# chengruiz/cusrl

Hardware: AMD Instinct MI355X
Metric: env_steps_per_sec (higher is better)
Workload: dtype f32; 1 GPU; synthetic continuous env 4096x obs48 x act12 per GPU, MLP(256,128) actor-critic, rollout_len=24, ppo preset (5 epochs x 4 minibatches, Adam lr 2e-4); envs_per_gpu=4096, parallelism=dp1, rccl_ranks=0, collectives=none (single process), hipgraph=True, fused_env=True, captured_env_steps=24, epoch_graph_updates=432, unjoined_steps_captured=20, autoreset=False

## Files before the change

### cusrl_amd/csrc/mlp_forward.hip

```cpp
#include "common.hpp"

namespace cusrl {

typedef float mfma_f32x4 __attribute__((ext_vector_type(4)));

constexpr int kMlpWaves = 4;
constexpr int kMlpThreads = kMlpWaves * kWave;
constexpr int kMlpRows = 16;

struct MlpForwardArgs {
    const float *x;
    const float *w1, *b1, *w2, *b2, *w3, *b3;
    float *out;
    const float *std;
    const float *eps;
    float *action, *logp, *std_out;
    int64_t rows;
    int K, A;
};

__device__ __forceinline__ float log_sqrt_2pi_f() { return 0.91893853320467274178f; }

__device__ __forceinline__ mfma_f32x4 relu4(mfma_f32x4 v) {
    v[0] = v[0] <= 0.f ? 0.f : v[0], v[1] = v[1] <= 0.f ? 0.f : v[1], v[2] = v[2] <= 0.f ? 0.f : v[2], v[3] = v[3] <= 0.f ? 0.f : v[3];
    return v;
}

template <int T1, int T2, int KB>
__global__ __launch_bounds__(kMlpThreads) void mlp2_forward_kernel(const MlpForwardArgs p) {
    constexpr int NT1 = kMlpWaves * T1;
    __shared__ float4 hidden[NT1][kWave];
    __shared__ float4 partial[kMlpWaves][kWave];
    const int lane = threadIdx.x & (kWave - 1), wave = threadIdx.x / kWave;
    const int i = lane & 15, kk = lane >> 4;
    const int K = p.K, A = p.A;
    constexpr int H1 = 16 * NT1, H2 = 16 * kMlpWaves * T2;
    const float4 zero4 = make_float4(0.f, 0.f, 0.f, 0.f);

    float4 a1[T1][KB], a2[T2][NT1], a3[T2];
    mfma_f32x4 c1[T1], c2[T2], c3;
#pragma unroll
    for (int t1 = 0; t1 < T1; ++t1) {
        const int n = 16 * (T1 * wave + t1);
#pragma unroll
        for (int t = 0; t < KB; ++t) {
            const int k = 16 * t + 4 * kk;
            const float4 v = *reinterpret_cast<const float4 *>(p.w1 + int64_t(n + i) * K + (k < K ? k : 0));
            a1[t1][t] = k < K ? v : zero4;
        }
        const float4 b = *reinterpret_cast<const float4 *>(p.b1 + n + 4 * kk);
        c1[t1] = mfma_f32x4{b.x, b.y, b.z, b.w};
    }
    const int64_t tiles = (p.rows + kMlpRows - 1) / kMlpRows;
    float4 ahead[KB];
    auto request = [&](int64_t tile) {
        const int64_t row = min(tile * kMlpRows + i, p.rows - 1);
#pragma unroll
        for (int t = 0; t < KB; ++t) {
            const int k = 16 * t + 4 * kk;
            ahead[t] = *reinterpret_cast<const float4 *>(p.x + row * K + (k < K ? k : 0));
        }
    };
    request(min(int64_t(blockIdx.x), tiles - 1));
#pragma unroll
    for (int t2 = 0; t2 < T2; ++t2) {
        const int n = 16 * (T2 * wave + t2);
#pragma unroll
        for (int t = 0; t < NT1; ++t) a2[t2][t] = *reinterpret_cast<const float4 *>(p.w2 + int64_t(n + i) * H1 + 16 * t + 4 * kk);
        const float4 b = *reinterpret_cast<const float4 *>(p.b2 + n + 4 * kk);
        c2[t2] = mfma_f32x4{b.x, b.y, b.z, b.w};
        const float4 v = *reinterpret_cast<const float4 *>(p.w3 + int64_t(i < A ? i : 0) * H2 + n + 4 * kk);
        a3[t2] = i < A ? v : zero4;
    }
    c3 = mfma_f32x4{0.f, 0.f, 0.f, 0.f};
    if (wave == 0 && p.b3) {
#pragma unroll
        for (int reg = 0; reg < 4; ++reg) c3[reg] = 4 * kk + reg < A ? p.b3[4 * kk + reg] : 0.f;
    }

    float sigma[4] = {1.f, 1.f, 1.f, 1.f}, noise[4] = {0.f, 0.f, 0.f, 0.f};
    const bool sampling = wave == 0 && p.eps != nullptr;
    if (sampling) {
#pragma unroll
        for (int reg = 0; reg < 4; ++reg) sigma[reg] = p.std[min(4 * kk + reg, A - 1)];
    }

    for (int64_t tile = blockIdx.x; tile < tiles; tile += gridDim.x) {
        const int64_t row0 = tile * kMlpRows;
        if (sampling) {
            const int64_t first = min(row0 + i, p.rows - 1) * A;
#pragma unroll
            for (int reg = 0; reg < 4; ++reg) noise[reg] = p.eps[first + min(4 * kk + reg, A - 1)];
        }
        float4 xb[KB];
#pragma unroll
        for (int t = 0; t < KB; ++t) xb[t] = 16 * t + 4 * kk < K ? ahead[t] : zero4;
        request(min(tile + gridDim.x, tiles - 1));
#pragma unroll
        for (int t1 = 0; t1 < T1; ++t1) {
            mfma_f32x4 acc = c1[t1];
#pragma unroll
            for (int t = 0; t < KB; ++t) {
                const float av[4] = {a1[t1][t].x, a1[t1][t].y, a1[t1][t].z, a1[t1][t].w};
                const float bv[4] = {xb[t].x, xb[t].y, xb[t].z, xb[t].w};
#pragma unroll
                for (int j = 0; j < 4; ++j) acc = __builtin_amdgcn_mfma_f32_16x16x4f32(av[j], bv[j], acc, 0, 0, 0);
            }
            acc = relu4(acc);
            hidden[T1 * wave + t1][lane] = make_float4(acc[0], acc[1], acc[2], acc[3]);
        }
        __syncthreads();
        mfma_f32x4 h2[T2];
#pragma unroll
        for (int t2 = 0; t2 < T2; ++t2) h2[t2] = c2[t2];
#pragma unroll
        for (int t = 0; t < NT1; ++t) {
            const float4 hb = hidden[t][lane];
            const float bv[4] = {hb.x, hb.y, hb.z, hb.w};
#pragma unroll
            for (int j = 0; j < 4; ++j)
#pragma unroll
                for (int t2 = 0; t2 < T2; ++t2) {
                    const float av = j == 0 ? a2[t2][t].x : j == 1 ? a2[t2][t].y : j == 2 ? a2[t2][t].z : a2[t2][t].w;
                    h2[t2] = __builtin_amdgcn_mfma_f32_16x16x4f32(av, bv[j], h2[t2], 0, 0, 0);
                }
        }
        mfma_f32x4 head = c3;
#pragma unroll
        for (int t2 = 0; t2 < T2; ++t2) {
            const mfma_f32x4 h = relu4(h2[t2]);
            const float av[4] = {a3[t2].x, a3[t2].y, a3[t2].z, a3[t2].w};
#pragma unroll
            for (int j = 0; j < 4; ++j) head = __builtin_amdgcn_mfma_f32_16x16x4f32(av[j], h[j], head, 0, 0, 0);
        }
        partial[wave][lane] = make_float4(head[0], head[1], head[2], head[3]);
        __syncthreads();
        if (wave == 0) {
            float4 sum = partial[0][lane];
#pragma unroll
            for (int w = 1; w < kMlpWaves; ++w) {
                const float4 v = partial[w][lane];
                sum.x += v.x, sum.y += v.y, sum.z += v.z, sum.w += v.w;
            }
            const bool live = row0 + i < p.rows;
            const int a0 = 4 * kk;
            const int64_t at = (row0 + i) * A + a0;
            const float mu[4] = {sum.x, sum.y, sum.z, sum.w};
            if (live && p.out) {
                if (A % 4 == 0) {
                    if (a0 < A) *reinterpret_cast<float4 *>(p.out + at) = sum;
                } else {
#pragma unroll
                    for (int reg = 0; reg < 4; ++reg)
                        if (a0 + reg < A) p.out[at + reg] = mu[reg];
                }
            }
            if (p.eps) {
                float term[4] = {0.f, 0.f, 0.f, 0.f};
#pragma unroll
                for (int reg = 0; reg < 4; ++reg) {
                    const int a = a0 + reg;
                    if (a < A) {
                        const float sg = sigma[reg];
                        const float act = mu[reg] + noise[reg] * sg;
                        const float diff = act - mu[reg];
                        term[reg] = -(diff * diff) / (2.0f * (sg * sg)) - logf(sg) - log_sqrt_2pi_f();
                        if (live) {
                            p.action[at + reg] = act;
                            if (p.std_out) p.std_out[at + reg] = sg;
                        }
                    }
                }
                float lp = 0.f;
#pragma unroll
                for (int src = 0; src < 4; ++src)
#pragma unroll
                    for (int reg = 0; reg < 4; ++reg) {
                        const float t = __shfl(term[reg], i + 16 * src, kWave);
                        if (4 * src + reg < A) lp += t;
                    }
                if (live && kk == 0) p.logp[row0 + i] = lp;
            }
        }
    }
}

template <int T1, int T2>
static int launch_mlp2(const MlpForwardArgs &p, int kb, dim3 grid, hipStream_t s) {
    switch (kb) {
        case 1: hipLaunchKernelGGL((mlp2_forward_kernel<T1, T2, 1>), grid, dim3(kMlpThreads), 0, s, p); break;
        case 2: hipLaunchKernelGGL((mlp2_forward_kernel<T1, T2, 2>), grid, dim3(kMlpThreads), 0, s, p); break;
        case 3: hipLaunchKernelGGL((mlp2_forward_kernel<T1, T2, 3>), grid, dim3(kMlpThreads), 0, s, p); break;
        case 4: hipLaunchKernelGGL((mlp2_forward_kernel<T1, T2, 4>), grid, dim3(kMlpThreads), 0, s, p); break;
        default: return CUSRL_E_UNSUPPORTED;
    }
    return launch_status();
}

}

using namespace cusrl;

extern "C" int cusrl_mlp2_forward_supported(int64_t in_features, int64_t hidden1, int64_t hidden2, int64_t out_features) {
    return in_features >= 4 && in_features % 4 == 0 && in_features <= 64 && (hidden1 == 128 || hidden1 == 256) &&
           (hidden2 == 64 || hidden2 == 128) && out_features >= 1 && out_features <= 16;
}

extern "C" int cusrl_mlp2_forward(const float *input, int64_t rows, int64_t in_features, const float *w1, const float *b1,
                                  int64_t hidden1, const float *w2, const float *b2, int64_t hidden2, const float *w3,
                                  const float *b3, int64_t out_features, float *output, const float *std, const float *eps,
                                  float *action, float *logp, float *std_out, void *stream) {
    if (rows < 0 || !input || !w1 || !b1 || !w2 || !b2 || !w3) return CUSRL_E_INVALID;
    if (rows == 0) return 0;
    if (!cusrl_mlp2_forward_supported(in_features, hidden1, hidden2, out_features)) return CUSRL_E_UNSUPPORTED;
    const bool sampling = eps != nullptr;
    if (sampling ? !(std && action && logp) : (std || action || logp || std_out)) return CUSRL_E_INVALID;
    if (!sampling && !output) return CUSRL_E_INVALID;
    if (!aligned(input, 16) || !aligned(w1, 16) || !aligned(b1, 16) || !aligned(w2, 16) || !aligned(b2, 16) || !aligned(w3, 16) ||
        (output && out_features % 4 == 0 && !aligned(output, 16)))
        return CUSRL_E_UNSUPPORTED;
    MlpForwardArgs p;
    p.x = input, p.w1 = w1, p.b1 = b1, p.w2 = w2, p.b2 = b2, p.w3 = w3, p.b3 = b3, p.out = output;
    p.std = std, p.eps = eps, p.action = action, p.logp = logp, p.std_out = std_out;
    p.rows = rows, p.K = int(in_features), p.A = int(out_features);
    const int64_t tiles = ceil_div(rows, kMlpRows);
    static int cus = 0;
    if (cus == 0) {
        int device = 0, count = 0;
        if (hipGetDevice(&device) != hipSuccess || hipDeviceGetAttribute(&count, hipDeviceAttributeMultiprocessorCount, device) != hipSuccess || count <= 0)
            count = 256;
        cus = count;
    }
    const dim3 grid(uint32_t(tiles < cus ? tiles : cus));
    const int kb = int(ceil_div(in_features, 16));
    hipStream_t s = as_stream(stream);
    if (hidden1 == 256 && hidden2 == 128) return launch_mlp2<4, 2>(p, kb, grid, s);
    if (hidden1 == 256 && hidden2 == 64) return launch_mlp2<4, 1>(p, kb, grid, s);
    if (hidden1 == 128 && hidden2 == 128) return launch_mlp2<2, 2>(p, kb, grid, s);
    return launch_mlp2<2, 1>(p, kb, grid, s);
}
```

### cusrl_amd/hook/on_policy/value.py

```python

from __future__ import annotations

import torch
from torch import Tensor, nn

from cusrl_amd import ops
from cusrl_amd.hook.on_policy.fused import FusedPpoObjective
from cusrl_amd.template.buffer import Buffer
from cusrl_amd.template.hook import Hook
from cusrl_amd.utils.misc import get_first
from cusrl_amd.utils.nest import map_nested

__all__ = ["ValueComputation", "ValueLoss"]


class ValueComputation(Hook):

    def __init__(self, *, termination_value: float = 0.0, bootstrap_truncated_states: bool = True,
                 defer_value: bool | None = None):
        super().__init__()
        self.termination_value = termination_value
        self.bootstrap_truncated_states = bootstrap_truncated_states
        self.defer_value = defer_value
        self._critic_memory = None
        self._value_pending = False
        self._auto_defer: bool | None = None
        self._replay_scratch: dict | None = None

    def init(self):
        if self.agent.environment_spec.final_state_is_missing:
            self.bootstrap_truncated_states = False

    def _deferred(self) -> bool:
        critic = self.agent.critic
        if getattr(critic, "is_recurrent", False) or self.agent.inference_mode:
            return False
        if self.defer_value is not None:
            return bool(self.defer_value)
        if self._auto_defer is None:
            self._auto_defer = self.agent.device.type == "cuda" and all(
                type(hook).__module__.startswith("cusrl_amd.") for hook in self.agent.hook if hook.active)
        return self._auto_defer

    def post_act(self, transition):
        if self._deferred():
            return
        state = get_first(transition, "state", "observation")
        with self.agent.autocast():
            value, next_memory = self.agent.critic(state, memory=self._critic_memory, sequential=False)
        transition["value"] = value
        transition["critic_memory"] = self._critic_memory
        transition["next_critic_memory"] = next_memory
        self._critic_memory = next_memory

    @property
    def post_step_device_free(self) -> bool:
        return self._deferred()

    def post_step(self, transition):
        if self._deferred():
            self._value_pending = True
            return
        self.agent.critic.reset_memory(self._critic_memory, transition["done"])

    def on_replay(self, phase):
        if phase == "step" and self._deferred():
            self._value_pending = True

    @torch.no_grad()
    def pre_update(self, buffer: Buffer):
        if self._value_pending and self._replayable(buffer):
            self._value_pending = False
            return self._pre_update_replayed(buffer)
        critic = self.agent.critic
        if self._value_pending:
            self._value_pending = False
            state: Tensor = get_first(buffer, "state", "observation")
            with self.agent.autocast():
                flat_value = critic.evaluate(state.flatten(0, 1))
            stacked = flat_value.float().view(*state.shape[:2], -1)
            buffer.field("value", stacked).copy_(stacked)
        value: Tensor = buffer["value"]
        next_value = buffer.field("next_value", value)
        next_state: Tensor = get_first(buffer, "next_state", "next_observation")
        terminated, truncated = buffer["terminated"], buffer["truncated"]
        T, N = value.shape[:2]

        with self.agent.autocast():
            last_value = critic.evaluate(next_state[-1], memory=self._critic_memory)
        counts = ops.next_value(
            value, terminated, truncated, last_value.float(), self.termination_value,
            truncated_uses_own_value=not self.bootstrap_truncated_states, out=next_value,
        )
        if not self.bootstrap_truncated_states:
            return
        slots, count = ops.compact_flags(truncated, counts)
        k = int(count.item())
        if k == 0:
            return
        slots = slots[:k]
        (truncated_next_state,) = ops.gather_rows([next_state], slots, T, N)
        next_memory = buffer.get("next_critic_memory")
        if next_memory is not None:
            next_memory = map_nested(lambda m: ops.gather_rows([m], slots, T, N)[0], next_memory)
        with self.agent.autocast():
            truncated_next_value = critic.evaluate(truncated_next_state, memory=next_memory)
        ops.scatter_rows(truncated_next_value.float(), slots, next_value)

    _MIN_BUCKET = 256

    def _replayable(self, buffer: Buffer) -> bool:
        agent = self.agent
        return (bool(getattr(agent, "compile", False)) and getattr(agent, "_graph_stream", None) is not None
                and "value" in buffer.storage and "next_value" in buffer.storage
                and buffer.get("next_critic_memory") is None and self._critic_memory is None)

    def _pre_update_replayed(self, buffer: Buffer):
        from cusrl_amd.template.graphs import GraphedRegion

        state: Tensor = get_first(buffer, "state", "observation")
        value = buffer.field("value", buffer.storage["value"])
        next_value = buffer.field("next_value", value)
        next_state: Tensor = get_first(buffer, "next_state", "next_observation")
        terminated, truncated = buffer["terminated"], buffer["truncated"]
        T, N = value.shape[:2]
        scratch = self._replay_scratch
        key = (buffer.layout_version, state.data_ptr(), next_state.data_ptr(), T, N)
        if scratch is None or scratch["key"] != key:
            scratch = self._replay_scratch = {"key": key, "slots": torch.zeros(T * N, dtype=torch.int64, device=value.device),
                                              "counters": (ops.HostCounter(), ops.HostCounter()), "parity": 0, "heads": {}, "tails": {}}
        parity = scratch["parity"] = scratch["parity"] ^ 1
        slots, counter = scratch["slots"], scratch["counters"][parity]
        compaction = scratch.get("compaction")
        if compaction is None:
            from cusrl_amd import _native

            blocks = max(int(_native.lib().cusrl_flag_blocks(T * N)), 1)
            compaction = scratch["compaction"] = {"n": T * N, "device": truncated.device, "indices": slots,
                                                  "counts": torch.empty(blocks, dtype=torch.int32, device=truncated.device)}
        critic, autocast = self.agent.critic, self.agent.autocast

        def head():
            if self.bootstrap_truncated_states:
                ops.compact_flags(truncated, None, counter.tensor, scratch=compaction)
            with autocast():
                flat_value = critic.evaluate(state.flatten(0, 1))
                last_value = critic.evaluate(next_state[-1])
            value.copy_(flat_value.float().view(T, N, -1))
            ops.next_value(value, terminated, truncated, last_value.float(), self.termination_value,
                           truncated_uses_own_value=not self.bootstrap_truncated_states, out=next_value)

        if parity not in scratch["heads"]:
            scratch["heads"][parity] = GraphedRegion(self.agent, head)
        counter.arm()
        scratch["heads"][parity].run(self.bootstrap_truncated_states, self.termination_value)
        if not self.bootstrap_truncated_states:
            return
        if (idle := getattr(self.agent, "run_while_waiting", None)) is not None:
            idle()
        k = counter.wait()
        if k == 0:
            return
        bucket = scratch.get("bucket", 0)
        if k > bucket:
            bucket = scratch["bucket"] = min(max(self._MIN_BUCKET, 1 << (2 * k - 1).bit_length()), T * N)

        def tail():
            (rows,) = ops.gather_rows([next_state], slots[:bucket], T, N)
            with autocast():
                bootstrap = critic.evaluate(rows)
            ops.scatter_rows(bootstrap.float(), slots[:bucket], next_value, counter.tensor)

        region = scratch["tails"].get((bucket, parity))
        if region is None:
            region = scratch["tails"][(bucket, parity)] = GraphedRegion(self.agent, tail)
        region.run(bucket)


def _clipped_value_loss(value: Tensor, curr_value: Tensor, return_: Tensor, loss_clip: float) -> Tensor:
    clipped = value + (curr_value - value).clamp(-loss_clip, loss_clip)
    return torch.max((curr_value - return_).square(), (clipped - return_).square()).mean()


class ValueLoss(Hook):
    def __init__(self, weight: float = 0.5, loss_clip: float | None = None):
        if weight <= 0:
            raise ValueError("'weight' must be positive")
        if loss_clip is not None and loss_clip <= 0:
            raise ValueError("'loss_clip' must be positive or None")
        super().__init__()
        self.weight: float = weight
        self.loss_clip: float | None = loss_clip
        self.register_mutable("weight")
        self.register_mutable("loss_clip")

    def objective(self, metadata, batch):
        state = get_first(batch, "state", "observation")
        memory, done = batch.get("critic_memory"), batch["done"]
        fused = FusedPpoObjective.current(self)
        branch = self.agent.step_context.critic_stream if fused is not None and not fused.split else None
        if branch is not None:
            main = torch.cuda.current_stream()
            separate = self.agent.separate_value_root and fused.unit_grad
            if separate:
                ret, old_value = batch["return"], (batch["value"] if self.loss_clip is not None else None)
            if not (separate and self.agent.step_context.batch_on_branch):
                branch.wait_stream(main)
            with torch.cuda.stream(branch):
                curr_value = self.agent.critic.evaluate(state, memory=memory, done=done)
                if separate:
                    terms = fused.evaluate_value(curr_value, old_value, ret, self.weight, self.loss_clip, branch)
            curr_value.record_stream(main)
            if separate:
                batch["curr_value"] = curr_value
                return terms
            fused.join(branch)
        else:
            curr_value = self.agent.critic.evaluate(state, memory=memory, done=done)
        batch["curr_value"] = curr_value
        if fused is not None:
            old_value = batch["value"] if self.loss_clip is not None else None
            return fused.add_value(curr_value, old_value, batch["return"], self.weight, self.loss_clip)
        if self.loss_clip is None:
            loss = nn.functional.mse_loss(batch["return"], curr_value)
        else:
            loss = _clipped_value_loss(batch["value"], curr_value, batch["return"], self.loss_clip)
        return {"value_loss": loss * self.weight}

    def post_objective(self, metadata, batch):
# ... 10 lines not shown
```

### cusrl_amd/ops/__init__.py

```python

from __future__ import annotations

import os
from collections.abc import Sequence

import torch

from cusrl_amd import _native
from cusrl_amd._native import Field, MirrorField, PackedField, check
from cusrl_amd.ops._common import (
    LaunchObserver, _checked, _f32, _flag, _modified_in_place, _observed, _ptr, _raw_stream, _row_bytes, _stream, require_device,
    set_launch_observer,
)
from cusrl_amd.ops.advantage import (
    adv_stats_finalize, col_stats, gae, merge_mean_var, next_value, normalize_, normalize_from_gathered_, normalize_from_partials_,
    packed_mean_var,
)
from cusrl_amd.ops.auxiliary import (
    accumulate_scalars_, action_smoothness_fwd_bwd, amp_prepare, amp_prepare_supported, amp_style_reward_, amp_style_reward_mean_, bce_pair_fwd_bwd,
    column_mse_fwd_bwd, column_table, masked_col_stats, mse_loss_fwd_bwd, nan_to_num_, normal_nll_bound, normal_nll_fwd_bwd,
    resolve_columns, reward_shaping_, rms_merge_, rms_normalize, rnd_reward_, sumsq_fwd_bwd,
)
from cusrl_amd.ops.buffer import (
    HostCounter, RecordPack, _row_elems, assign_rows, buffer_push, compact_flags, gather_rows, gather_rows_packed, make_push_table,
    push_table, scatter_rows, splice_rows, window_indices,
)
from cusrl_amd.ops.gradient import (
    DeferredColumns, adam_norm_workspace, adam_step, adam_step_normed, adam_step_window, assemble_gradients, clip_grad_norm_,
    grad_sumsq, sum_slabs,
)
from cusrl_amd.ops.graph import graph_census, graph_replace_memsets
from cusrl_amd.ops.loss import (
    LOSS_DEFER, DeferredLoss, _optional_rows, categorical_policy_stats, categorical_terms_bwd, categorical_terms_fwd, policy_stats,
    policy_terms_bwd, policy_terms_fwd, ppo_loss_accepts_std_vector, ppo_loss_categorical_fwd_bwd, ppo_loss_fwd_bwd,
    value_loss_fwd_bwd,
)
from cusrl_amd.ops.mlp import (
    _HEAD_PAD, input_layer_backward, input_layer_supported, mlp2_forward, mlp2_forward_supported, narrow_linear_backward,
    narrow_linear_forward, narrow_linear_forward_supported, narrow_linear_supported, relu_backward_bias,
)
from cusrl_amd.ops.recurrent import (
    gru_bias_partial_rows, gru_bias_partials_supported, gru_gates_backward, gru_gates_forward, lstm_gates_backward,
    lstm_gates_forward, rnn_cell_backward, rnn_cell_forward,
)
from cusrl_amd.ops.rollout import (
    PendingStepEpilogue, categorical_sample_logp, episode_stats, normal_sample_logp, step_epilogue, synthetic_env_step,
)
from cusrl_amd.ops.symmetry import (
    _mirror_table, _rows_2d, mirror_mse_fwd_bwd, mirror_rows, mirror_rows_bwd, symmetric_head_bwd, symmetric_head_fwd,
    symmetric_head_sample, symmetric_head_supported, symmetrize_mean_var_,
)
```

### cusrl_amd/ops/buffer.py

```python

from __future__ import annotations

from collections.abc import Sequence

import torch

from cusrl_amd import _native
from cusrl_amd._native import Field, PackedField
from cusrl_amd.ops._common import _checked, _flag, _modified_in_place, _observed, _ptr, _row_bytes, _stream, require_device


def buffer_push(pairs: Sequence[tuple[torch.Tensor, torch.Tensor]], cursor: int, parallelism: int) -> None:
    for start in range(0, len(pairs), _native.MAX_FIELDS):
        chunk = pairs[start : start + _native.MAX_FIELDS]
        table = (Field * len(chunk))()
        for i, (step, storage) in enumerate(chunk):
            table[i].src = step.data_ptr()
            table[i].dst = storage.data_ptr()
            table[i].row_bytes = _row_bytes(step, 1)
        _observed("cusrl_buffer_push", table, len(chunk), cursor, parallelism,
                nbytes=lambda: sum(2 * step.numel() * step.element_size() for step, _ in chunk))


def make_push_table(leaves: Sequence[tuple[torch.Tensor, tuple]]):
# ... 256 lines not shown
    if count_out is not None:
        if count_out.dtype != torch.int32 or count_out.numel() != 1 or not (count_out.is_cuda or count_out.is_pinned()):
            raise TypeError("'count_out' must be a 1-element int32 tensor on the device or in pinned host memory")
        count = count_out
    else:
        count = torch.empty(1, dtype=torch.int32, device=flags.device)
    _checked.cusrl_compact_flags(flags.data_ptr(), n, block_counts.data_ptr(), int(recount), indices.data_ptr(), count.data_ptr(), _stream())
    return indices, count


def assign_rows(dst: torch.Tensor, indices: torch.Tensor, src: torch.Tensor) -> None:
    require_device(src, "src"), require_device(dst, "dst"), require_device(indices, "indices")
    if src.dtype != dst.dtype or indices.dtype != torch.int64 or not dst.is_contiguous() or src.shape[1:] != dst.shape[1:]:
        raise TypeError("assign_rows: dtype/layout mismatch")
    K = indices.numel()
    if K == 0:
        return
    if src.shape[0] != K:
        raise ValueError("assign_rows: one source row per index is required")
    src, indices = src.contiguous(), indices.contiguous()
    _checked.cusrl_scatter_rows(src.data_ptr(), indices.data_ptr(), dst.data_ptr(), K, _row_bytes(src, 1), None, _stream())
    _modified_in_place(dst)


def splice_rows(src: torch.Tensor, init: torch.Tensor, indices: torch.Tensor, count: torch.Tensor, done: torch.Tensor,
                dst: torch.Tensor) -> torch.Tensor:
    for tensor, name in ((src, "src"), (init, "init"), (indices, "indices"), (count, "count"), (done, "done"), (dst, "dst")):
        require_device(tensor, name)
    N = src.shape[0]
    if (src.dtype != dst.dtype or init.dtype != dst.dtype or src.shape != dst.shape or init.shape != dst.shape
            or not (src.is_contiguous() and init.is_contiguous() and dst.is_contiguous())):
        raise TypeError("splice_rows: src, init and dst must be contiguous tensors of one shape and dtype")
    if indices.dtype != torch.int64 or indices.numel() < N or count.dtype != torch.int32 or count.numel() != 1 or done.numel() != N:
        raise TypeError("splice_rows: indices int64[>= N], count int32[1], done [N] flags are required")
    if dst.data_ptr() in (src.data_ptr(), init.data_ptr()):
        raise ValueError("splice_rows: dst must not alias src or init")
    done = _flag(done, "done")
    _checked.cusrl_splice_rows(src.data_ptr(), init.data_ptr(), indices.data_ptr(), count.data_ptr(), done.data_ptr(),
            dst.data_ptr(), N, _row_bytes(src, 1), _stream())
    _modified_in_place(dst)
    return dst


class HostCounter:

    def __init__(self):
        self.tensor = torch.empty(1, dtype=torch.int32).pin_memory()
        self._view = self.tensor.numpy()

    def arm(self) -> torch.Tensor:
        self._view[0] = -1
        return self.tensor

    def wait(self, timeout: float = 0.01) -> int:
        import time

        view, deadline = self._view, None
        while True:
            value = int(view[0])
            if value >= 0:
                return value
            if deadline is None:
                deadline = time.perf_counter() + timeout
            elif time.perf_counter() > deadline:
                torch.cuda.current_stream().synchronize()
                value = int(view[0])
                if value < 0:
                    raise RuntimeError("HostCounter: the kernel retired without publishing its count")
                return value


def scatter_rows(src: torch.Tensor, indices: torch.Tensor, dst: torch.Tensor, count: torch.Tensor | None = None) -> None:
    require_device(src, "src"), require_device(dst, "dst"), require_device(indices, "indices")
    if count is not None and (count.dtype != torch.int32 or count.numel() != 1 or not (count.is_cuda or count.is_pinned())):
        raise TypeError("'count' must be a 1-element int32 tensor on the device or in pinned host memory")
    if src.dtype != dst.dtype or indices.dtype != torch.int64 or not dst.is_contiguous():
        raise TypeError("scatter_rows: dtype/layout mismatch")
    src, indices = src.contiguous(), indices.contiguous()
    K = indices.numel()
    if K == 0:
        return
    _checked.cusrl_scatter_rows(src.data_ptr(), indices.data_ptr(), dst.data_ptr(), K, _row_bytes(src, 1), _ptr(count), _stream())
    _modified_in_place(dst)
```

### cusrl_amd/ops/mlp.py

```python

from __future__ import annotations

import torch

from cusrl_amd import _native
from cusrl_amd.ops._common import _checked, _f32, _observed, _ptr, _stream
from cusrl_amd.ops.gradient import DeferredColumns


def relu_backward_bias(grad_output: torch.Tensor, output: torch.Tensor | None, defer: bool = False):
    grad_output = _f32(grad_output, "grad_output")
    H = grad_output.shape[-1]
    rows = grad_output.numel() // H
    lib = _native.lib()
    num_partials = max(int(lib.cusrl_colsum_num_partials(rows, H)), 1)
    partials = torch.empty((num_partials, H), dtype=torch.float32, device=grad_output.device)
    chunkable = H % 4 == 0 and H // 4 <= 256 and 256 % (H // 4) == 0
    defer = defer and chunkable and grad_output.data_ptr() % 16 == 0 and (output is None or output.data_ptr() % 16 == 0)
    colsum = None if defer else torch.empty(H, dtype=torch.float32, device=grad_output.device)
    if output is None:
        grad_in, out_ptr, in_ptr = grad_output, None, None
    else:
        output = _f32(output, "output")
        grad_in = torch.empty_like(grad_output)
        out_ptr, in_ptr = output.data_ptr(), grad_in.data_ptr()
    _checked.cusrl_relu_bwd_colsum(grad_output.data_ptr(), out_ptr, in_ptr, partials.data_ptr(), _ptr(colsum), rows, H, _stream())
    return grad_in, (DeferredColumns(partials, num_partials, H, 0, H) if colsum is None else colsum)


def input_layer_supported(grad_output: torch.Tensor, output: torch.Tensor | None, input: torch.Tensor, weight: torch.Tensor) -> bool:
    H, K = weight.shape
    tensors = [grad_output, input] + ([] if output is None else [output])
    return (bool(_native.lib().cusrl_input_layer_supported(K, H)) and input.dim() == 2 and grad_output.shape == (input.shape[0], H)
            and all(t.is_cuda and t.dtype == torch.float32 and t.is_contiguous() and t.data_ptr() % 16 == 0 for t in tensors)
            and (output is None or output.shape == grad_output.shape) and input.shape[0] > 0)


def input_layer_backward(grad_output: torch.Tensor, output: torch.Tensor | None, input: torch.Tensor) -> tuple[torch.Tensor, torch.Tensor]:
    grad_output, input = _f32(grad_output, "grad_output"), _f32(input, "input")
    rows, K = input.shape
    H = grad_output.shape[-1]
    lib = _native.lib()
    dev = input.device
    width = H * K + H
    partials = torch.empty((int(lib.cusrl_input_layer_row_blocks(rows, H)), width), dtype=torch.float32, device=dev)
    grads = torch.empty(width, dtype=torch.float32, device=dev)
    _observed("cusrl_input_layer_bwd", grad_output.data_ptr(), _ptr(None if output is None else _f32(output, "output")),
            input.data_ptr(), rows, K, H, partials.data_ptr(), grads.data_ptr(),
            nbytes=lambda: rows * 4 * ((2 if output is not None else 1) * H + K) + (partials.numel() * 2 + width) * 4)
    return grads[: H * K].view(H, K), grads[H * K :]


_HEAD_PAD = 16


def narrow_linear_supported(in_features: int, out_features: int) -> bool:
    return bool(_native.lib().cusrl_narrow_linear_supported(in_features, out_features))


# ... 2 lines not shown
            and weight.dtype == torch.float32 and input.is_contiguous() and weight.is_contiguous() and input.shape[0] > 0
            and input.data_ptr() % 16 == 0 and weight.data_ptr() % 16 == 0 and narrow_linear_supported(weight.shape[1], 1))


def narrow_linear_forward(input: torch.Tensor, weight: torch.Tensor, bias: torch.Tensor | None) -> torch.Tensor:
    input, weight = _f32(input, "input"), _f32(weight, "weight")
    rows, K = input.shape
    out = torch.empty((rows, 1), dtype=torch.float32, device=input.device)
    _checked.cusrl_narrow_linear_fwd(input.data_ptr(), weight.data_ptr(), _ptr(None if bias is None else _f32(bias, "bias")),
            out.data_ptr(), rows, K, 1, _stream())
    return out


def mlp2_forward_supported(input: torch.Tensor, layers) -> bool:
    w1, b1, w2, b2, w3, b3 = layers
    tensors = [input, w1, b1, w2, b2, w3] + ([b3] if b3 is not None else [])
    if input.dim() != 2 or input.shape[0] == 0 or any(
            (not t.is_cuda) or t.dtype != torch.float32 or (not t.is_contiguous()) or t.data_ptr() % 16 for t in tensors):
        return False
    if w1.dim() != 2 or w2.dim() != 2 or w3.dim() != 2 or w1.shape[1] != input.shape[1] or w2.shape[1] != w1.shape[0] \
            or w3.shape[1] != w2.shape[0] or b1.numel() != w1.shape[0] or b2.numel() != w2.shape[0] \
            or (b3 is not None and b3.numel() != w3.shape[0]):
        return False
    return bool(_native.lib().cusrl_mlp2_forward_supported(w1.shape[1], w1.shape[0], w2.shape[0], w3.shape[0]))


def mlp2_forward(input: torch.Tensor, layers, std: torch.Tensor | None = None, eps: torch.Tensor | None = None,
                 repeat_std: bool = True):
    w1, b1, w2, b2, w3, b3 = layers
    input = _f32(input, "input")
    rows, K = input.shape
    out_features = w3.shape[0]
    out = torch.empty((rows, out_features), dtype=torch.float32, device=input.device)
    sampling = eps is not None
    action = logp = repeated = None
    if sampling:
        std, eps = _f32(std, "std"), _f32(eps, "eps")
        if std.numel() != out_features or eps.shape != out.shape:
            raise ValueError("mlp2_forward: one std per output and one eps per output element are required")
        action = torch.empty_like(out)
        logp = torch.empty((rows, 1), dtype=torch.float32, device=input.device)
        repeated = torch.empty_like(out) if repeat_std else None
    _observed(
        "cusrl_mlp2_forward", input.data_ptr(), rows, K, w1.data_ptr(), b1.data_ptr(), w1.shape[0], w2.data_ptr(),
        b2.data_ptr(), w2.shape[0], w3.data_ptr(), _ptr(b3), out_features, out.data_ptr(),
        _ptr(std) if sampling else None, _ptr(eps), _ptr(action), _ptr(logp), _ptr(repeated),
        nbytes=lambda: rows * 4 * (K + out_features * (4 if sampling else 1)) + 4 * (w1.numel() + w2.numel() + w3.numel()),
    )
    if sampling:
        return action, logp, out, repeated
    return out


def narrow_linear_backward(grad_output: torch.Tensor, input: torch.Tensor, weight: torch.Tensor,
                           need_input_grad: bool = True, relu_input: bool = False, defer: bool = False):
    grad_output, input, weight = _f32(grad_output, "grad_output"), _f32(input, "input"), _f32(weight, "weight")
    O, K = weight.shape
    rows = input.shape[0]
    lib = _native.lib()
    dev = input.device
    grad_input = torch.empty_like(input) if need_input_grad else None
    width = (O + 1) * K + _HEAD_PAD
    num_partials = int(lib.cusrl_narrow_linear_num_partials(rows))
    partials = torch.empty((num_partials, width), dtype=torch.float32, device=dev)
    packed = None if defer else torch.empty(width, dtype=torch.float32, device=dev)
    _checked.cusrl_narrow_linear_bwd(grad_output.data_ptr(), input.data_ptr(), weight.data_ptr(), _ptr(grad_input),
            partials.data_ptr(), _ptr(packed), rows, K, O, int(relu_input), _stream())
    if defer:
        window = lambda column, numel: DeferredColumns(partials, num_partials, width, column, numel)
        return grad_input, window(0, O * K), window((O + 1) * K, O), (window(O * K, K) if relu_input else None)
    colsum = packed[O * K : (O + 1) * K] if relu_input else None
    return grad_input, packed[: O * K].view(O, K), packed[(O + 1) * K : (O + 1) * K + O], colsum
```

### cusrl_amd/template/actor_critic.py

```python

from __future__ import annotations

from collections.abc import Callable, Iterable, Mapping, Sequence
from contextlib import contextmanager
from dataclasses import dataclass
from typing import Any

import torch

from cusrl_amd.nn.actor import Actor, Value
from cusrl_amd.nn.module import collect_split_weight_grads, register_unit_gradient
from cusrl_amd.template.agent import Agent, AgentFactory, preserve_io_format
from cusrl_amd.template.buffer import Buffer, Sampler
from cusrl_amd.template.environment import EnvironmentSpec
from cusrl_amd.template.hook import Hook, HookComposite
from cusrl_amd.template.optimizer import OptimizerFactory, build_optimizer
from cusrl_amd.utils import switches
from cusrl_amd.utils.config import CONFIG
from cusrl_amd.utils.distributed import FlatGradients, UnjoinedStep, broadcast_parameters, reduce_gradients

__all__ = ["ActorCritic", "ActorCriticFactory", "HookList", "StepContext", "StepPlan", "plan_step"]


def _hashable(value):
# ... 307 lines not shown
                def while_waiting():
                    early.draw(len(early) - 1)
                    if self._graphed_epochs is not None:
                        self._graphed_epochs.prepare(early)

                self._while_waiting = while_waiting
        try:
            self.hook.pre_update(self.buffer)
        finally:
            self._while_waiting = None
        with self._training_mode():
            graphed = self._graphable()
            if graphed:
                from cusrl_amd.template.graphs import GraphedTrainStep

                from cusrl_amd.template.graphs import GraphedEpochs

                drawn = early if early is not None else self._draw_epochs()
                if drawn is not None and self._graphed_epochs is None:
                    self._graphed_epochs = GraphedEpochs(self)
                steps = () if drawn is not None and self._graphed_epochs.run(drawn) else (
                    self._iter_drawn(drawn) if drawn is not None else self.sampler.iter_indices(self.buffer))
                for metadata, indices in steps:
                    key = self._step_key(metadata, indices.numel())
                    if (step := self._graphed_steps.get(key)) is None:
                        if self._graph_key_reads != len(self._metadata_reads):
                            self._graph_key_reads = len(self._metadata_reads)
                            width = len(key)
                            for stale in [k for k in self._graphed_steps if len(k) != width]:
                                self._graphed_steps.pop(stale).flush_metrics()
                        step = self._graphed_steps[key] = GraphedTrainStep(self, key[0], key[1])
                        budget = self.sampler.num_epochs * (self.sampler.num_mini_batches if isinstance(self.sampler.num_mini_batches, int)
                                                            else max(self.sampler.num_mini_batches)) if hasattr(self.sampler, "num_epochs") else 0
                        if budget and len(self._graphed_steps) > budget and not self._graph_budget_warned:
                            self._graph_budget_warned = True
                            self.warn(f"{len(self._graphed_steps)} minibatch-step graphs for {budget} steps per update: a hook reads "
                                      f"metadata whose values keep changing ({sorted(self._metadata_reads)}); every distinct value is "
                                      "its own capture")
                    step.run(metadata, indices)
                if drawn is not None:
                    if self._minibatches_done is None:
                        self._minibatches_done = torch.cuda.Event()
                    self._minibatches_done.record(torch.cuda.current_stream())
                for step in self._graphed_steps.values():
                    step.flush_metrics()
                if self._graphed_epochs is not None:
                    self._graphed_epochs.flush_metrics()
            else:
                for metadata, batch in self.sampler(self.buffer):
                    self._train_step(metadata, batch)
        self.hook.post_update()
        self.hook.apply_schedule(self.iteration + 1)
        return super().update()

    def run_while_waiting(self) -> None:
        pending, self._while_waiting = self._while_waiting, None
        if pending is not None:
            pending()

    def _graphable(self) -> bool:
        if not (self.compile and hasattr(self.sampler, "iter_indices")) or self.actor.is_recurrent or self.critic.is_recurrent:
            return False
        from cusrl_amd.template.graphs import eager_phases

        return "objective" not in eager_phases(self)

    def _draws_early(self) -> bool:
        return self._graphable() and all(type(hook).__module__.startswith("cusrl_amd.") for hook in self.hook if hook.active)

    def _draw_epochs(self, prepare: bool = True):
        from cusrl_amd.template.graphs import epoch_graphs_enabled

        if not (epoch_graphs_enabled() and hasattr(self.sampler, "draw_epochs")):
            return None
        return self.sampler.draw_epochs(self.buffer, after=self._minibatches_done, prepare=prepare)

    def _step_key(self, metadata, numel: int) -> tuple:
        key = (metadata["mini_batch_index"], metadata["temporal"], numel)
        if self._metadata_reads:
            key += tuple((name, _hashable(metadata.get(name))) for name in sorted(self._metadata_reads)
                         if name not in ("mini_batch_index", "temporal"))
        return key

    @staticmethod
    def _iter_drawn(drawn):
        for epoch, row in enumerate(drawn.plan):
            drawn.wait(epoch)
            for metadata, lo, hi in row:
                yield dict(metadata), drawn.permutations[epoch, lo:hi]

    def _zero_grad(self):
        if self.flat_optimizer is not None:
            self.flat_optimizer.discard_pending_clip()
        if self.flat_gradients is None:
            self.optimizer.zero_grad()
        elif not self.flat_gradients.intact():
            self.flat_gradients.attach()

    def _backward(self, loss):
        flat = self.flat_gradients
        roots = list(loss) if isinstance(loss, (list, tuple)) else [loss]
        if len(roots) > 1:
            roots = [t for t in roots if isinstance(t, torch.Tensor) and t.requires_grad] or roots[:1]
        if flat is None:
            total = roots[0]
            for term in roots[1:]:
# ... 152 lines not shown
```

### include/cusrl_hip.h

```cpp
#ifndef CUSRL_HIP_H
#define CUSRL_HIP_H

#include <stdint.h>

#ifdef __cplusplus
extern "C" {
#endif

#define CUSRL_ABI_VERSION 7
#define CUSRL_MAX_FIELDS 24
#define CUSRL_MAX_PACKED 16
#define CUSRL_MAX_RECORD_BYTES 1024
#define CUSRL_MAX_MIRROR_FIELDS 24
#define CUSRL_MAX_SYMMETRIZE_CHANNELS 4096
#define CUSRL_MAX_SYMMETRIC_HEAD_ACTIONS 64

#define CUSRL_E_INVALID (-1)
#define CUSRL_E_TOO_MANY (-2)
#define CUSRL_E_UNSUPPORTED (-3)
#define CUSRL_E_COMM (-4)

typedef struct {
    const void *src;
    void *dst;
// ... 127 lines not shown
                        float *episode_rew, float *episode_len, float *ring_rew, float *ring_len, uint64_t *num_episodes,
                        double *step_reward_sum, int64_t *indices_out, int32_t *count_out, int64_t N, int64_t D, int64_t R,
                        int parity, void *stream);
int64_t cusrl_step_epilogue_max_envs(void);
int cusrl_step_epilogue_push(const float *reward, const uint8_t *terminated, const uint8_t *truncated, uint8_t *done_out,
                             float *episode_rew, float *episode_len, float *ring_rew, float *ring_len, uint64_t *num_episodes,
                             double *step_reward_sum, int64_t *indices_out, int32_t *count_out, int64_t N, int64_t D, int64_t R,
                             int parity, const cusrl_field_t *fields, int n_fields, int done_field, int64_t cursor,
                             void *stream);

int cusrl_policy_stats(const float *old_mean, const float *old_std, const float *new_mean, const float *new_std,
                       const float *action, const float *old_logp, const float *advantage, int64_t B, int64_t A,
                       int64_t D, double *partials, float *out, void *stream);
int64_t cusrl_policy_stats_num_partials(int64_t B);
int cusrl_categorical_policy_stats(const float *old_logits, const float *new_logits, const float *action,
                                   const float *old_logp, const float *advantage, int64_t B, int64_t A, int64_t D,
                                   double *partials, float *out, void *stream);

int cusrl_policy_terms_fwd(const float *mean, const float *std, int64_t std_rows, const float *action,
                           const float *old_logp, int64_t B, int64_t A, float *logp_out, float *entropy_out,
                           float *logp_ratio_out, float *ratio_out, void *stream);
int cusrl_policy_terms_bwd(const float *mean, const float *std, int64_t std_rows, const float *action, const float *ratio,
                           const float *g_logp, const float *g_entropy, const float *g_logp_ratio, const float *g_ratio,
                           int64_t B, int64_t A, float *d_mean, float *d_std, float *d_std_partials, void *stream);
int64_t cusrl_policy_terms_std_partial_rows(int64_t B);
int cusrl_categorical_terms_fwd(const float *logits, const float *action, const float *old_logp, int64_t B, int64_t A,
                                float *logp_out, float *entropy_out, float *logp_ratio_out, float *ratio_out, void *stream);
int cusrl_categorical_terms_bwd(const float *logits, const float *action, const float *ratio, const float *g_logp,
                                const float *g_entropy, const float *g_logp_ratio, const float *g_ratio, int64_t B,
                                int64_t A, float *d_logits, void *stream);

int cusrl_relu_bwd_colsum(const float *grad, const float *output, float *grad_in, float *partials, float *colsum,
                          int64_t rows, int64_t H, void *stream);
int64_t cusrl_colsum_num_partials(int64_t rows, int64_t H);

int cusrl_input_layer_bwd(const float *grad_out, const float *output, const float *input, int64_t rows, int64_t in_features,
                          int64_t out_features, float *partials, float *grads, void *stream);
int cusrl_input_layer_supported(int64_t in_features, int64_t out_features);
int64_t cusrl_input_layer_row_blocks(int64_t rows, int64_t out_features);

int cusrl_narrow_linear_bwd(const float *grad_out, const float *input, const float *weight, float *grad_input,
                            float *partials, float *packed, int64_t rows, int64_t in_features, int64_t out_features,
                            int relu_input, void *stream);
int64_t cusrl_narrow_linear_num_partials(int64_t rows);
int cusrl_narrow_linear_supported(int64_t in_features, int64_t out_features);
int cusrl_narrow_linear_fwd(const float *input, const float *weight, const float *bias, float *output, int64_t rows,
                            int64_t in_features, int64_t out_features, void *stream);

int cusrl_mlp2_forward(const float *input, int64_t rows, int64_t in_features, const float *w1, const float *b1, int64_t hidden1,
                       const float *w2, const float *b2, int64_t hidden2, const float *w3, const float *b3, int64_t out_features,
                       float *output, const float *std, const float *eps, float *action, float *logp, float *std_out,
                       void *stream);
int cusrl_mlp2_forward_supported(int64_t in_features, int64_t hidden1, int64_t hidden2, int64_t out_features);

int cusrl_clip_grad_norm(float *grad, int64_t n, float max_norm, double *partials, float *norm_out, void *stream);
int64_t cusrl_clip_grad_norm_num_partials(int64_t n);

typedef struct {
    const void *src;
    int64_t offset;
    int64_t numel;
    int64_t splits;
    int64_t row_stride;
} cusrl_grad_piece_t;
int cusrl_assemble_gradients(const cusrl_grad_piece_t *pieces, int64_t num_pieces, float *flat, double *sumsq_partials,
                             void *stream);
int64_t cusrl_assemble_gradients_blocks(const cusrl_grad_piece_t *pieces, int64_t num_pieces);

int cusrl_grad_sumsq(const float *grad, int64_t n, double *partials, void *stream);

int cusrl_adam_step(float *param, const float *grad, float *exp_avg, float *exp_avg_sq, float *step, const float *lr,
                    int64_t n, double beta1, double beta2, double eps, double weight_decay, int decoupled_weight_decay,
                    int maximize, const double *clip_partials, int64_t num_clip_partials, float max_norm,
                    float *norm_out, float *norm_accumulator, uint32_t *ticket, void *stream);

int cusrl_adam_step_window(float *param, const float *grad, float *exp_avg, float *exp_avg_sq, float *step, const float *lr,
                           int64_t n, double beta1, double beta2, double eps, double weight_decay, int decoupled_weight_decay,
                           int maximize, const double *clip_partials_a, int64_t num_a, const double *clip_partials_b,
                           int64_t num_b, float max_norm, float *norm_out, float *norm_accumulator, float *step_mirror,
                           uint32_t *ticket, void *stream);

int cusrl_adam_step_normed(float *param, const float *grad, float *exp_avg, float *exp_avg_sq, float *step, const float *lr,
                           int64_t n, double beta1, double beta2, double eps, double weight_decay, int decoupled_weight_decay,
                           int maximize, const float *norm_grad, int64_t norm_n, void *workspace, float max_norm, float *norm_out,
                           float *norm_accumulator, float *step_mirror, uint32_t *ticket, void *stream);
int64_t cusrl_adam_step_normed_workspace_bytes(void);

int cusrl_masked_col_stats(const float *x, const uint8_t *mask, int64_t rows, int64_t C, double *partials,
                           float *batch_mean, float *batch_var, double *batch_count, void *stream);
int64_t cusrl_masked_stats_num_partials(int64_t rows, int64_t C);

int cusrl_rms_merge(float *mean, float *var, float *std, double *count, const float *batch_mean,
                    const float *batch_var, const double *batch_count, float eps, double max_count, int64_t C,
                    void *stream);

int cusrl_rms_normalize(const float *x, const float *mean, const float *std, float clamp, float *out, int64_t rows,
                        int64_t C, void *stream);

int cusrl_sequence_count(const uint8_t *done, int64_t L, int64_t N, int32_t *env_prefix, int32_t *block_totals,
                         int32_t *num_sequences, void *stream);
int64_t cusrl_sequence_blocks(int64_t N);
int cusrl_sequence_layout(const uint8_t *done, int64_t L, int64_t N, const int32_t *env_prefix,
                          const int32_t *block_totals, int64_t Ns, int64_t *dest, int64_t *first_seq, uint8_t *mask,
                          int64_t *seq_lengths, int64_t *last_seq, void *stream);
int cusrl_gather_memory(const void *memory, const int64_t *last_seq, const uint8_t *done_last, void *out, int64_t N,
                        int64_t row_bytes, void *stream);
// ... 98 lines not shown
```

Measured before the change: 21.04 million env-steps/s.

## Bootstrap truncated values with device-counted indexed MLP kernel, avoiding host wait

```diff
diff --git a/cusrl_amd/csrc/mlp_forward.hip b/cusrl_amd/csrc/mlp_forward.hip
--- a/cusrl_amd/csrc/mlp_forward.hip
+++ b/cusrl_amd/csrc/mlp_forward.hip
@@ -17,6 +17,8 @@
     float *action, *logp, *std_out;
     int64_t rows;
     int K, A;
+    const int64_t *row_index;
+    const int32_t *row_count;
 };
 
 __device__ __forceinline__ float log_sqrt_2pi_f() { return 0.91893853320467274178f; }
@@ -26,7 +28,7 @@
     return v;
 }
 
-template <int T1, int T2, int KB>
+template <int T1, int T2, int KB, bool Indexed>
 __global__ __launch_bounds__(kMlpThreads) void mlp2_forward_kernel(const MlpForwardArgs p) {
     constexpr int NT1 = kMlpWaves * T1;
     __shared__ float4 hidden[NT1][kWave];
@@ -36,6 +38,12 @@
     const int K = p.K, A = p.A;
     constexpr int H1 = 16 * NT1, H2 = 16 * kMlpWaves * T2;
     const float4 zero4 = make_float4(0.f, 0.f, 0.f, 0.f);
+    int64_t rows = p.rows;
+    if constexpr (Indexed) {
+        const int64_t count = *p.row_count;
+        rows = count < 0 ? 0 : count < rows ? count : rows;
+        if (int64_t(blockIdx.x) * kMlpRows >= rows) return;
+    }
 
     float4 a1[T1][KB], a2[T2][NT1], a3[T2];
     mfma_f32x4 c1[T1], c2[T2], c3;
@@ -51,10 +59,11 @@
         const float4 b = *reinterpret_cast<const float4 *>(p.b1 + n + 4 * kk);
         c1[t1] = mfma_f32x4{b.x, b.y, b.z, b.w};
     }
-    const int64_t tiles = (p.rows + kMlpRows - 1) / kMlpRows;
+    const int64_t tiles = (rows + kMlpRows - 1) / kMlpRows;
     float4 ahead[KB];
     auto request = [&](int64_t tile) {
-        const int64_t row = min(tile * kMlpRows + i, p.rows - 1);
+        int64_t row = min(tile * kMlpRows + i, rows - 1);
+        if constexpr (Indexed) row = p.row_index[row];
 #pragma unroll
         for (int t = 0; t < KB; ++t) {
             const int k = 16 * t + 4 * kk;
@@ -79,7 +88,7 @@
     }
 
     float sigma[4] = {1.f, 1.f, 1.f, 1.f}, noise[4] = {0.f, 0.f, 0.f, 0.f};
-    const bool sampling = wave == 0 && p.eps != nullptr;
+    const bool sampling = !Indexed && wave == 0 && p.eps != nullptr;
     if (sampling) {
 #pragma unroll
         for (int reg = 0; reg < 4; ++reg) sigma[reg] = p.std[min(4 * kk + reg, A - 1)];
@@ -88,10 +97,12 @@
     for (int64_t tile = blockIdx.x; tile < tiles; tile += gridDim.x) {
         const int64_t row0 = tile * kMlpRows;
         if (sampling) {
-            const int64_t first = min(row0 + i, p.rows - 1) * A;
+            const int64_t first = min(row0 + i, rows - 1) * A;
 #pragma unroll
             for (int reg = 0; reg < 4; ++reg) noise[reg] = p.eps[first + min(4 * kk + reg, A - 1)];
         }
+        int64_t dest = 0;
+        if constexpr (Indexed) dest = wave == 0 ? p.row_index[min(row0 + i, rows - 1)] : 0;
         float4 xb[KB];
 #pragma unroll
         for (int t = 0; t < KB; ++t) xb[t] = 16 * t + 4 * kk < K ? ahead[t] : zero4;
@@ -142,9 +153,9 @@
                 const float4 v = partial[w][lane];
                 sum.x += v.x, sum.y += v.y, sum.z += v.z, sum.w += v.w;
             }
-            const bool live = row0 + i < p.rows;
+            const bool live = row0 + i < rows;
             const int a0 = 4 * kk;
-            const int64_t at = (row0 + i) * A + a0;
+            const int64_t at = (Indexed ? dest : row0 + i) * A + a0;
             const float mu[4] = {sum.x, sum.y, sum.z, sum.w};
             if (live && p.out) {
                 if (A % 4 == 0) {
@@ -155,7 +166,7 @@
                         if (a0 + reg < A) p.out[at + reg] = mu[reg];
                 }
             }
-            if (p.eps) {
+            if (!Indexed && p.eps) {
                 float term[4] = {0.f, 0.f, 0.f, 0.f};
 #pragma unroll
                 for (int reg = 0; reg < 4; ++reg) {
@@ -185,16 +196,36 @@
     }
 }
 
-template <int T1, int T2>
+template <int T1, int T2, bool Indexed>
 static int launch_mlp2(const MlpForwardArgs &p, int kb, dim3 grid, hipStream_t s) {
     switch (kb) {
-        case 1: hipLaunchKernelGGL((mlp2_forward_kernel<T1, T2, 1>), grid, dim3(kMlpThreads), 0, s, p); break;
-        case 2: hipLaunchKernelGGL((mlp2_forward_kernel<T1, T2, 2>), grid, dim3(kMlpThreads), 0, s, p); break;
-        case 3: hipLaunchKernelGGL((mlp2_forward_kernel<T1, T2, 3>), grid, dim3(kMlpThreads), 0, s, p); break;
-        case 4: hipLaunchKernelGGL((mlp2_forward_kernel<T1, T2, 4>), grid, dim3(kMlpThreads), 0, s, p); break;
+        case 1: hipLaunchKernelGGL((mlp2_forward_kernel<T1, T2, 1, Indexed>), grid, dim3(kMlpThreads), 0, s, p); break;
+        case 2: hipLaunchKernelGGL((mlp2_forward_kernel<T1, T2, 2, Indexed>), grid, dim3(kMlpThreads), 0, s, p); break;
+        case 3: hipLaunchKernelGGL((mlp2_forward_kernel<T1, T2, 3, Indexed>), grid, dim3(kMlpThreads), 0, s, p); break;
+        case 4: hipLaunchKernelGGL((mlp2_forward_kernel<T1, T2, 4, Indexed>), grid, dim3(kMlpThreads), 0, s, p); break;
         default: return CUSRL_E_UNSUPPORTED;
     }
     return launch_status();
+}
+
+template <bool Indexed>
+static int dispatch_mlp2(const MlpForwardArgs &p, int64_t hidden1, int64_t hidden2, dim3 grid, hipStream_t s) {
+    const int kb = int(ceil_div(int64_t(p.K), 16));
+    if (hidden1 == 256 && hidden2 == 128) return launch_mlp2<4, 2, Indexed>(p, kb, grid, s);
+    if (hidden1 == 256 && hidden2 == 64) return launch_mlp2<4, 1, Indexed>(p, kb, grid, s);
+    if (hidden1 == 128 && hidden2 == 128) return launch_mlp2<2, 2, Indexed>(p, kb, grid, s);
+    return launch_mlp2<2, 1, Indexed>(p, kb, grid, s);
+}
+
+static dim3 mlp2_grid(int64_t tiles) {
+    static int cus = 0;
+    if (cus == 0) {
+        int device = 0, count = 0;
+        if (hipGetDevice(&device) != hipSuccess || hipDeviceGetAttribute(&count, hipDeviceAttributeMultiprocessorCount, device) != hipSuccess || count <= 0)
+            count = 256;
+        cus = count;
+    }
+    return dim3(uint32_t(tiles < cus ? tiles : cus));
 }
 
 }
@@ -223,19 +254,27 @@
     p.x = input, p.w1 = w1, p.b1 = b1, p.w2 = w2, p.b2 = b2, p.w3 = w3, p.b3 = b3, p.out = output;
     p.std = std, p.eps = eps, p.action = action, p.logp = logp, p.std_out = std_out;
     p.rows = rows, p.K = int(in_features), p.A = int(out_features);
-    const int64_t tiles = ceil_div(rows, kMlpRows);
-    static int cus = 0;
-    if (cus == 0) {
-        int device = 0, count = 0;
-        if (hipGetDevice(&device) != hipSuccess || hipDeviceGetAttribute(&count, hipDeviceAttributeMultiprocessorCount, device) != hipSuccess || count <= 0)
-            count = 256;
-        cus = count;
-    }
-    const dim3 grid(uint32_t(tiles < cus ? tiles : cus));
-    const int kb = int(ceil_div(in_features, 16));
-    hipStream_t s = as_stream(stream);
-    if (hidden1 == 256 && hidden2 == 128) return launch_mlp2<4, 2>(p, kb, grid, s);
-    if (hidden1 == 256 && hidden2 == 64) return launch_mlp2<4, 1>(p, kb, grid, s);
-    if (hidden1 == 128 && hidden2 == 128) return launch_mlp2<2, 2>(p, kb, grid, s);
-    return launch_mlp2<2, 1>(p, kb, grid, s);
-}
+    p.row_index = nullptr, p.row_count = nullptr;
+    return dispatch_mlp2<false>(p, hidden1, hidden2, mlp2_grid(ceil_div(rows, kMlpRows)), as_stream(stream));
+}
+
+extern "C" int cusrl_mlp2_forward_rows(const float *input, int64_t table_rows, int64_t in_features, const float *w1, const float *b1,
+                                       int64_t hidden1, const float *w2, const float *b2, int64_t hidden2, const float *w3,
+                                       const float *b3, int64_t out_features, const int64_t *row_index, const int32_t *row_count,
+                                       int64_t grid_rows, float *output, void *stream) {
+    if (table_rows < 0 || grid_rows < 0 || !input || !w1 || !b1 || !w2 || !b2 || !w3 || !row_index || !row_count || !output)
+        return CUSRL_E_INVALID;
+    if (table_rows == 0) return 0;
+    if (!cusrl_mlp2_forward_supported(in_features, hidden1, hidden2, out_features)) return CUSRL_E_UNSUPPORTED;
+    if (!aligned(input, 16) || !aligned(w1, 16) || !aligned(b1, 16) || !aligned(w2, 16) || !aligned(b2, 16) || !aligned(w3, 16) ||
+        (out_features % 4 == 0 && !aligned(output, 16)) || !aligned(row_index, 8) || !aligned(row_count, 4))
+        return CUSRL_E_UNSUPPORTED;
+    MlpForwardArgs p;
+    p.x = input, p.w1 = w1, p.b1 = b1, p.w2 = w2, p.b2 = b2, p.w3 = w3, p.b3 = b3, p.out = output;
+    p.std = nullptr, p.eps = nullptr, p.action = nullptr, p.logp = nullptr, p.std_out = nullptr;
+    p.rows = table_rows, p.K = int(in_features), p.A = int(out_features);
+    p.row_index = row_index, p.row_count = row_count;
+    const int64_t hinted = grid_rows < table_rows ? grid_rows : table_rows;
+    const int64_t tiles = ceil_div(hinted > 0 ? hinted : 1, kMlpRows);
+    return dispatch_mlp2<true>(p, hidden1, hidden2, mlp2_grid(tiles), as_stream(stream));
+}
diff --git a/cusrl_amd/hook/on_policy/value.py b/cusrl_amd/hook/on_policy/value.py
--- a/cusrl_amd/hook/on_policy/value.py
+++ b/cusrl_amd/hook/on_policy/value.py
@@ -17,11 +17,14 @@
 class ValueComputation(Hook):
 
     def __init__(self, *, termination_value: float = 0.0, bootstrap_truncated_states: bool = True,
-                 defer_value: bool | None = None):
+                 defer_value: bool | None = None, device_counted_tail: bool = True):
         super().__init__()
         self.termination_value = termination_value
         self.bootstrap_truncated_states = bootstrap_truncated_states
         self.defer_value = defer_value
+        self.device_counted_tail = device_counted_tail
+        self.device_counted_tails = 0
+        self._blocked = True
         self._critic_memory = None
         self._value_pending = False
         self._auto_defer: bool | None = None
@@ -72,6 +75,7 @@
         if self._value_pending and self._replayable(buffer):
             self._value_pending = False
             return self._pre_update_replayed(buffer)
+        self._blocked = True
         critic = self.agent.critic
         if self._value_pending:
             self._value_pending = False
@@ -109,6 +113,20 @@
 
     _MIN_BUCKET = 256
 
+    def _tail_layers(self, next_state: Tensor):
+        critic = self.agent.critic
+        if (not self.device_counted_tail or not getattr(critic, "fused_inference", False) or getattr(critic, "action_aware", False)
+                or getattr(critic, "backbone_kwargs", None) or not hasattr(critic, "value_head") or next_state.dim() != 3):
+            return None
+        from cusrl_amd.nn.module import fused_inference_layers
+
+        with self.agent.autocast():
+            return fused_inference_layers(critic.backbone, critic.value_head, next_state.flatten(0, 1))
+
+    @property
+    def update_blocks_on_device(self) -> bool:
+        return self._blocked
+
     def _replayable(self, buffer: Buffer) -> bool:
         agent = self.agent
         return (bool(getattr(agent, "compile", False)) and getattr(agent, "_graph_stream", None) is not None
@@ -129,6 +147,8 @@
         if scratch is None or scratch["key"] != key:
             scratch = self._replay_scratch = {"key": key, "slots": torch.zeros(T * N, dtype=torch.int64, device=value.device),
                                               "counters": (ops.HostCounter(), ops.HostCounter()), "parity": 0, "heads": {}, "tails": {}}
+            for fresh in scratch["counters"]:
+                fresh.arm()
         parity = scratch["parity"] = scratch["parity"] ^ 1
         slots, counter = scratch["slots"], scratch["counters"][parity]
         compaction = scratch.get("compaction")
@@ -139,6 +159,14 @@
             compaction = scratch["compaction"] = {"n": T * N, "device": truncated.device, "indices": slots,
                                                   "counts": torch.empty(blocks, dtype=torch.int32, device=truncated.device)}
         critic, autocast = self.agent.critic, self.agent.autocast
+        layers = self._tail_layers(next_state) if self.bootstrap_truncated_states else None
+        device_counted = layers is not None
+        if device_counted != scratch.get("device_counted", False):
+            if not device_counted:
+                torch.cuda.current_stream().synchronize()
+            scratch["tails"].clear()
+        scratch["device_counted"] = device_counted
+        self._blocked = self.bootstrap_truncated_states and not device_counted
 
         def head():
             if self.bootstrap_truncated_states:
@@ -152,10 +180,13 @@
 
         if parity not in scratch["heads"]:
             scratch["heads"][parity] = GraphedRegion(self.agent, head)
-        counter.arm()
+        if not device_counted:
+            counter.arm()
         scratch["heads"][parity].run(self.bootstrap_truncated_states, self.termination_value)
         if not self.bootstrap_truncated_states:
             return
+        if device_counted:
+            return self._device_counted_tail(scratch, counter, parity, layers, next_state, next_value, T * N)
         if (idle := getattr(self.agent, "run_while_waiting", None)) is not None:
             idle()
         k = counter.wait()
@@ -175,6 +206,27 @@
         if region is None:
             region = scratch["tails"][(bucket, parity)] = GraphedRegion(self.agent, tail)
         region.run(bucket)
+
+    def _device_counted_tail(self, scratch: dict, counter, parity: int, layers, next_state: Tensor, next_value: Tensor, rows: int):
+        from cusrl_amd.template.graphs import GraphedRegion
+
+        k = max(max(other.peek() for other in scratch["counters"]), 0)
+        bucket = scratch.get("bucket", 0)
+        if k > bucket or bucket == 0:
+            bucket = scratch["bucket"] = min(max(self._MIN_BUCKET, 1 << (2 * k - 1).bit_length()), rows)
+        slots = scratch["slots"]
+        table, out = next_state.flatten(0, 1), next_value.view(rows, -1)
+
+        def tail():
+            ops.mlp2_forward_rows(table, layers, slots, counter.tensor, bucket, out)
+
+        region = scratch["tails"].get((bucket, parity))
+        if region is None:
+            region = scratch["tails"][(bucket, parity)] = GraphedRegion(self.agent, tail)
+        region.run(bucket)
+        self.device_counted_tails += 1
+        if (idle := getattr(self.agent, "run_while_waiting", None)) is not None:
+            idle()
 
 
 def _clipped_value_loss(value: Tensor, curr_value: Tensor, return_: Tensor, loss_clip: float) -> Tensor:
diff --git a/cusrl_amd/ops/__init__.py b/cusrl_amd/ops/__init__.py
--- a/cusrl_amd/ops/__init__.py
+++ b/cusrl_amd/ops/__init__.py
@@ -36,7 +36,8 @@
     value_loss_fwd_bwd,
 )
 from cusrl_amd.ops.mlp import (
-    _HEAD_PAD, input_layer_backward, input_layer_supported, mlp2_forward, mlp2_forward_supported, narrow_linear_backward,
+    _HEAD_PAD, input_layer_backward, input_layer_supported, mlp2_forward, mlp2_forward_rows, mlp2_forward_supported,
+    narrow_linear_backward,
     narrow_linear_forward, narrow_linear_forward_supported, narrow_linear_supported, relu_backward_bias,
 )
 from cusrl_amd.ops.recurrent import (
diff --git a/cusrl_amd/ops/buffer.py b/cusrl_amd/ops/buffer.py
--- a/cusrl_amd/ops/buffer.py
+++ b/cusrl_amd/ops/buffer.py
@@ -332,6 +332,9 @@
         self._view[0] = -1
         return self.tensor
 
+    def peek(self) -> int:
+        return int(self._view[0])
+
     def wait(self, timeout: float = 0.01) -> int:
         import time
 
diff --git a/cusrl_amd/ops/mlp.py b/cusrl_amd/ops/mlp.py
--- a/cusrl_amd/ops/mlp.py
+++ b/cusrl_amd/ops/mlp.py
@@ -4,7 +4,7 @@
 import torch
 
 from cusrl_amd import _native
-from cusrl_amd.ops._common import _checked, _f32, _observed, _ptr, _stream
+from cusrl_amd.ops._common import _checked, _f32, _modified_in_place, _observed, _ptr, _stream, require_device
 from cusrl_amd.ops.gradient import DeferredColumns
 
 
@@ -113,6 +113,32 @@
     return out
 
 
+def mlp2_forward_rows(input: torch.Tensor, layers, row_index: torch.Tensor, row_count: torch.Tensor, grid_rows: int,
+                      out: torch.Tensor) -> torch.Tensor:
+    w1, b1, w2, b2, w3, b3 = layers
+    input = _f32(input, "input")
+    require_device(out, "out"), require_device(row_index, "row_index")
+    table_rows, K = input.shape
+    out_features = w3.shape[0]
+    if out.dtype != torch.float32 or not out.is_contiguous() or out.numel() != table_rows * out_features:
+        raise TypeError("mlp2_forward_rows: 'out' must be a contiguous float32 table of one row per input row")
+    if row_index.dtype != torch.int64 or not row_index.is_contiguous() or row_index.numel() > table_rows:
+        raise TypeError("mlp2_forward_rows: 'row_index' must be contiguous int64 with at most one entry per table row")
+    if row_count.dtype != torch.int32 or row_count.numel() != 1 or not (row_count.is_cuda or row_count.is_pinned()):
+        raise TypeError("'row_count' must be a 1-element int32 tensor on the device or in pinned host memory")
+    if table_rows == 0 or row_index.numel() == 0:
+        return out
+    rows = row_index.numel()
+    _observed(
+        "cusrl_mlp2_forward_rows", input.data_ptr(), rows, K, w1.data_ptr(), b1.data_ptr(), w1.shape[0], w2.data_ptr(),
+        b2.data_ptr(), w2.shape[0], w3.data_ptr(), _ptr(b3), out_features, row_index.data_ptr(), row_count.data_ptr(),
+        max(int(grid_rows), 0), out.data_ptr(),
+        nbytes=lambda: int(grid_rows) * 4 * (K + out_features + 2) + 4 * (w1.numel() + w2.numel() + w3.numel()),
+    )
+    _modified_in_place(out)
+    return out
+
+
 def narrow_linear_backward(grad_output: torch.Tensor, input: torch.Tensor, weight: torch.Tensor,
                            need_input_grad: bool = True, relu_input: bool = False, defer: bool = False):
     grad_output, input, weight = _f32(grad_output, "grad_output"), _f32(input, "input"), _f32(weight, "weight")
diff --git a/cusrl_amd/template/actor_critic.py b/cusrl_amd/template/actor_critic.py
--- a/cusrl_amd/template/actor_critic.py
+++ b/cusrl_amd/template/actor_critic.py
@@ -383,6 +383,11 @@
         self.hook.post_update()
         self.hook.apply_schedule(self.iteration + 1)
         return super().update()
+
+    @property
+    def update_is_nonblocking(self) -> bool:
+        declared = [bool(hook.update_blocks_on_device) for hook in self.hook if hook.active and hasattr(hook, "update_blocks_on_device")]
+        return bool(self.compile) and bool(declared) and not any(declared)
 
     def run_while_waiting(self) -> None:
         pending, self._while_waiting = self._while_waiting, None
diff --git a/include/cusrl_hip.h b/include/cusrl_hip.h
--- a/include/cusrl_hip.h
+++ b/include/cusrl_hip.h
@@ -203,6 +203,10 @@
                        float *output, const float *std, const float *eps, float *action, float *logp, float *std_out,
                        void *stream);
 int cusrl_mlp2_forward_supported(int64_t in_features, int64_t hidden1, int64_t hidden2, int64_t out_features);
+int cusrl_mlp2_forward_rows(const float *input, int64_t table_rows, int64_t in_features, const float *w1, const float *b1,
+                            int64_t hidden1, const float *w2, const float *b2, int64_t hidden2, const float *w3, const float *b3,
+                            int64_t out_features, const int64_t *row_index, const int32_t *row_count, int64_t grid_rows,
+                            float *output, void *stream);
 
 int cusrl_clip_grad_norm(float *grad, int64_t n, float max_norm, double *partials, float *norm_out, void *stream);
 int64_t cusrl_clip_grad_norm_num_partials(int64_t n);
```

New measurement: 20.74 million env-steps/s. 0.986x the previous value.
